# jrobine/actor-critic

Hardware: AMD Instinct MI355X
Metric: env-steps/sec (whole node) + ACKTR update ms, Breakout 84x84x4 (higher is better)
Workload: dtype fp32

## Files before the change

actor-critic_amd/actorcritic/_lib.py:

```python

import ctypes
import os

import torch

_HERE = os.path.dirname(os.path.abspath(__file__))
LIB_PATH = os.path.join(os.path.dirname(_HERE), 'libacmi.so')
if os.environ.get('ACMI_LIB'):
    LIB_PATH = os.environ['ACMI_LIB']

c_int = ctypes.c_int
c_i64 = ctypes.c_int64
c_u32 = ctypes.c_uint32
c_float = ctypes.c_float
c_vp = ctypes.c_void_p


class AcmiError(RuntimeError):
    """A libacmi entry point returned a non-zero status."""


class Net(ctypes.Structure):
    _fields_ = [('num_actions', c_int), ('conv3_filters', c_int), ('params', c_vp), ('conv_prep', c_vp),
                ('gemm_mode', c_int), ('forward_mode', c_int), ('conv_stats_mode', c_int)]
# ... 102 lines not shown
    'acmi_diag_segments': (c_int, [c_vp, c_vp, c_vp, c_int, c_vp, c_vp, c_vp]),
    'acmi_a2c_loss_ws_floats': (c_i64, [c_int]),
    'acmi_a2c_loss': (c_int, [c_vp, c_int, c_vp, c_vp, c_vp, c_vp, c_int, c_int, c_float, c_float, c_float,
                              c_vp, c_int, c_vp, c_vp, c_vp]),
    'acmi_ppo_loss_ws_floats': (c_i64, [c_int]),
    'acmi_ppo_loss': (c_int, [c_vp, c_int, c_vp, c_vp, c_vp, c_vp, c_vp, c_vp, c_int, c_int, c_float, c_float,
                              c_float, c_float, c_float, c_vp, c_int, c_vp, c_vp, c_vp, c_vp]),
    'acmi_gather_rows': (c_int, [c_vp, c_i64, c_i64, c_vp, c_i64, c_vp, c_i64, c_int, ctypes.POINTER(c_vp),
                                 ctypes.POINTER(c_vp), c_vp, c_vp]),
    'acmi_backward_ws_floats': (c_i64, [c_int, c_int, c_int]),
    'acmi_backward': (c_int, [ctypes.POINTER(Net), c_vp, c_i64, c_int, ctypes.POINTER(Acts),
                              ctypes.POINTER(Bwd), c_vp, c_vp, c_vp, c_i64, c_vp]),
    'acmi_kfac_output_stats': (c_int, [ctypes.POINTER(Net), c_int, ctypes.POINTER(Acts), ctypes.POINTER(Bwd),
                                       c_u32, c_u32, c_u32, c_vp, c_vp, c_i64, c_vp]),
    'acmi_backward_stacked': (c_int, [ctypes.POINTER(Net), c_vp, c_i64, c_int, ctypes.POINTER(Acts),
                                      ctypes.POINTER(Bwd), c_vp, c_vp, c_vp, c_i64, ctypes.POINTER(Bwd), c_u32, c_u32,
                                      c_u32, c_vp, c_i64, c_vp]),
    'acmi_kfac_output_stats_finish': (c_int, [ctypes.POINTER(Net), c_int, ctypes.POINTER(Acts), ctypes.POINTER(Bwd),
                                              c_vp, c_vp, c_i64, c_vp]),
    'acmi_debug_ws_flushes': (c_int, []),
    'acmi_debug_convt2': (c_int, [ctypes.POINTER(Net), c_int, c_vp, c_vp, c_vp, c_vp, c_int, c_vp, c_vp, c_vp, c_vp,
                                  c_vp]),
    'acmi_debug_convt2_form': (c_int, [c_int]),
    'acmi_kfac_ema': (c_int, [c_vp, c_vp, c_vp, c_i64, c_float, c_float, c_float, c_vp]),
    'acmi_kfac_inverse_layout': (c_int, [c_int, c_int, ctypes.POINTER(c_i64), ctypes.POINTER(c_i64)]),
    'acmi_kfac_inverse_floats': (c_i64, [c_int, c_int]),
    'acmi_kfac_inverse_ws_doubles': (c_i64, [c_int, c_int]),
    'acmi_kfac_inverse': (c_int, [c_int, c_int, c_vp, c_float, c_int, c_vp, c_vp, c_vp]),
    'acmi_kfac_eig_ws_doubles': (c_i64, [c_int, c_int]),
    'acmi_kfac_eigvals': (c_int, [c_int, c_int, c_vp, c_vp, c_vp, c_vp]),
    'acmi_kfac_step_ws_floats': (c_i64, [c_int, c_int]),
    'acmi_kfac_step': (c_int, [c_int, c_int, c_vp, c_vp, c_vp, c_vp, c_float, c_float, c_float, c_vp, c_vp,
                               c_vp, c_vp]),
    'acmi_opt_ws_floats': (c_i64, [c_i64]),
    'acmi_momentum_apply': (c_int, [c_vp, c_vp, c_vp, c_i64, c_float, c_float, c_float, c_vp, c_vp, c_vp]),
    'acmi_rmsprop_apply': (c_int, [c_vp, c_vp, c_vp, c_vp, c_i64, c_float, c_float, c_float, c_float, c_float,
                                   c_vp, c_vp, c_vp]),
    'acmi_adam_apply': (c_int, [c_vp, c_vp, c_vp, c_vp, c_i64, c_float, c_float, c_float, c_float, c_float,
                                c_vp, c_vp, c_vp]),
    'acmi_env_reset': (c_int, [ctypes.POINTER(EnvState), c_int, c_int, c_u32, c_vp, c_i64, c_vp]),
    'acmi_env_step': (c_int, [ctypes.POINTER(EnvState), c_int, c_int, c_u32, c_vp, c_vp, c_i64, c_vp, c_i64,
                              c_vp, c_vp, c_vp, c_i64, c_vp]),
    'acmi_game_state_ints': (c_int, []),
    'acmi_game_state_bytes': (c_i64, []),
    'acmi_game_reset': (c_int, [ctypes.POINTER(GameState), c_int, c_int, c_u32, c_vp, c_i64, c_vp]),
    'acmi_game_step': (c_int, [ctypes.POINTER(GameState), c_int, c_int, c_u32, c_vp, c_vp, c_i64, c_vp, c_i64,
# ... 99 lines not shown
```

actor-critic_amd/csrc/gemm.hpp:

```cpp
#pragma once

#include <algorithm>
#include <type_traits>

#include "gemm_ops.hpp"


namespace acmi {

typedef float f32x16 __attribute__((ext_vector_type(16)));

template <int BM, int BN, int BK, int WTM, int WTN>
struct Tile {
  static constexpr int WAVES_M = BM / (32 * WTM);
  static constexpr int WAVES_N = BN / (32 * WTN);
  static_assert(WAVES_M * WAVES_N == 4, "4 waves per block");
  static_assert(BK % 2 == 0 && BK % 4 == 0, "");
  static_assert((BM * BK / 4) % 256 == 0 && (BN * BK / 4) % 256 == 0,
                "staging must split evenly over 256 threads");
};

template <class T, class = void>
struct has_vec4 : std::false_type {};
template <class T>
// ... 424 lines not shown
    if (relu) v = fmaxf(v, 0.f);
    out[(long long)i * ld + j] = v;
  }
};

template <bool MASK = false>
struct EpiReluGrad {
  float* out;
  const float* act;
  long long ld;
  unsigned* amax = nullptr;
  __device__ __forceinline__ float aux(int i, int j) const {
    const long long e = (long long)i * ld + j;
    if constexpr (MASK) return (float)((reinterpret_cast<const uint32_t*>(act)[e >> 5] >> (e & 31)) & 1u);
    else return act[e];
  }
  __device__ __forceinline__ float store(int i, int j, float v, float x) const {
    const float o = x > 0.f ? v : 0.f;
    out[(long long)i * ld + j] = o;
    return o;
  }
};

template <int IH, int IW, int S, int CIN, bool MASK = false>
struct EpiConvT {
  static constexpr bool VEC4 = true;
  static constexpr bool LDS_T = true;
  static_assert(CIN % 4 == 0, "channel runs of 4");
  float* out;
  const float* act;
  unsigned* amax = nullptr;
  __device__ __forceinline__ long long offset(int i, int j) const {
    constexpr int PH = IH / S, PW = IW / S, L = PH * PW;
    const uint32_t img = (uint32_t)j / L;
    const uint32_t p = (uint32_t)j - img * L;
    const uint32_t ihp = p / PW;
    const uint32_t iwp = p - ihp * PW;
    const int ph = i / (S * CIN);
    const int rem = i - ph * (S * CIN);
    const int pw = rem / CIN;
    const int ci = rem - pw * CIN;
    return (((long long)img * IH + (S * ihp + ph)) * IW + (S * iwp + pw)) * CIN + ci;
  }
  __device__ __forceinline__ float4 aux4(int i0, int j) const {
    const long long e = offset(i0, j);
    if constexpr (MASK) {
// ... 114 lines not shown
```

actor-critic_amd/csrc/gemm3.hpp:

```cpp
#pragma once

#include "f16x2.hpp"
#include "gemm.hpp"
#include "symred3.hpp"

namespace acmi {

template <int RB>
__device__ __forceinline__ int sw_rows(int slot, int k) {
  const int q = k & 3;
  if constexpr (RB >= 256) return slot ^ (8 * q);
  else if constexpr (RB == 128) return slot ^ (8 * ((q >> 1) & 1));
  else return slot;
}

template <int BK>
__device__ __forceinline__ int sw_kc(int c, int i) {
  if constexpr (BK == 16) return c ^ ((i >> 3) & 1);
  else return c ^ ((i >> 2) & 3);
}

template <int BM, int BN, int BK, int NP = 3>
constexpr int gemm3_lds_bytes() {
  return 2 * NP * (BM + BN) * BK * 2;
// ... 26 lines not shown
    *reinterpret_cast<uint2*>(s + off) = h;
    *reinterpret_cast<uint2*>(s + PART + off) = m;
    if constexpr (NP == 3) *reinterpret_cast<uint2*>(s + 2 * PART + off) = l;
  }
  __device__ __forceinline__ static int frag_off(int lane, int ks, int x0) {
    if constexpr (KC) {
      const int x = x0 + (lane & 31);
      return x * RB + 16 * sw_kc<BK>(2 * ks + (lane >> 5), x);
    } else {
      const int q = (lane >> 2) & 3, p = lane & 3, g = (lane >> 4) & 1, kh = lane >> 5;
      const int k = 16 * ks + 8 * kh + q;
      return k * RB + 8 * sw_rows<RB>((x0 >> 2) + 4 * g + p, k);
    }
  }
  __device__ __forceinline__ static bf16x8 frag(const char* part, int off) {
    if constexpr (KC) {
      return __builtin_bit_cast(bf16x8, *reinterpret_cast<const uint4*>(part + off));
    } else {
      return cat8(ds_tr16(part + off), ds_tr16(part + off + 4 * RB));
    }
  }
};

template <int BM, int BN, int BK, int WTM, int WTN, bool SPLITK, bool COLSUM, class OpA, class OpB,
          class Epi, bool F16 = false>
__global__ __launch_bounds__(256)
__attribute__((amdgpu_waves_per_eu(gemm3_blocks_per_cu<BM, BN, BK, 3>())))
void gemm3_kernel(OpA opA, OpB opB, Epi epi, int I, int J, int K, int k_chunk, int sym_cols,
                  const unsigned* amax_a = nullptr, const unsigned* amax_b = nullptr) {
  using TL = Tile<BM, BN, BK, WTM, WTN>;
  static_assert(BK == 16 || BK == 32, "BK 16 or 32");
  static_assert(!COLSUM || !OpB::KCONTIG, "column sums need an i-contiguous B");
  constexpr int NP = F16 ? 2 : 3;
  using IA = X3Image<OpA::KCONTIG, BM, BK, NP>;
  using IB = X3Image<OpB::KCONTIG, BN, BK, NP>;
  float sa = 1.f, sb = 1.f;
  if constexpr (F16) {
    sa = f16x2_scale_of_bits(amax_a);
    sb = f16x2_scale_of_bits(amax_b);
  }
  int bx = blockIdx.x, by = blockIdx.y, bz = blockIdx.z;
  if constexpr (SPLITK) {
    const int tx = (I + BM - 1) / BM, ty = (J + BN - 1) / BN;
    const int ssym = sym_cols > 0 ? sym_cols / BN : 0;
    int live = 0;
    for (int x = 0; x < tx; ++x) live += ty - min(x * BM / BN, ssym);
    const int total = gridDim.x;
    const int b = blockIdx.x;
    const int xcd = b & 7, base = total >> 3, rem = total & 7;
    const int l = xcd * base + min(xcd, rem) + (b >> 3);
// ... 214 lines not shown
    __syncthreads();
    if (bx == 0 && wm == 0) {
#pragma unroll
      for (int tn = 0; tn < WTN; ++tn) {
        const int c = wn * WTN * 32 + tn * 32 + (lane & 31);
        float t = 0.f;
        for (int r = 0; r < KT; ++r) t += cs[r * BN + c];
        const int j = j0 + c;
        if (lane < 32 && j < J) epi.colsum(j, t);
      }
    }
    __syncthreads();
  }

  if constexpr (F16) {
    const float inv = 1.0f / (sa * sb);
#pragma unroll
    for (int a = 0; a < WTM; ++a)
#pragma unroll
      for (int b = 0; b < WTN; ++b)
#pragma unroll
        for (int r = 0; r < 16; ++r) acc[a][b][r] *= inv;
  }
  if constexpr (has_ldst<Epi>::value && 2 * (IA::BYTES + IB::BYTES) >= 4 * 32 * 36 * 4) {
    __syncthreads();
    store_tile_lds<WTM, WTN>(epi, acc, i0 + wm * WTM * 32, j0 + wn * WTN * 32, lane,
                             reinterpret_cast<float*>(lds) + wave * 32 * 36, I, J);
  } else {
    store_tile<WTM, WTN>(epi, acc, i0 + wm * WTM * 32, j0 + wn * WTN * 32, lane, I, J);
  }
}

template <int BM, int BN, int BK, int WTM, int WTN, bool SPLITK, bool COLSUM, class OpA, class OpB,
          class Epi>
inline void launch_gemm3(const OpA& a, const OpB& b, const Epi& e, int I, int J, int K, int zdim,
                         int k_chunk, hipStream_t s, int sym_cols = 0) {
  dim3 grid(cdiv(I, BM), cdiv(J, BN), zdim);
  if (SPLITK) grid = dim3(live_tiles<BM, BN>(I, J, sym_cols) * zdim);
  hipLaunchKernelGGL((gemm3_kernel<BM, BN, BK, WTM, WTN, SPLITK, COLSUM, OpA, OpB, Epi>), grid,
                     dim3(256), 0, s, a, b, e, I, J, K, k_chunk, sym_cols, nullptr, nullptr);
}

template <int BM, int BN, int BK, int WTM, int WTN, class OpA, class OpB, class Epi>
inline void launch_gemm3_f16(const OpA& a, const OpB& b, const Epi& e, int I, int J, int K,
                             const unsigned* amax_a, const unsigned* amax_b, hipStream_t s) {
  hipLaunchKernelGGL((gemm3_kernel<BM, BN, BK, WTM, WTN, false, false, OpA, OpB, Epi, true>),
                     dim3(cdiv(I, BM), cdiv(J, BN), 1), dim3(256), 0, s, a, b, e, I, J, K, 0, 0, amax_a,
// ... 24 lines not shown
```

actor-critic_amd/csrc/net.hip:

```cpp
#include <math.h>
#include <stdlib.h>
#include <stdarg.h>
#include <stdio.h>
#include <string.h>

#include <atomic>
#include <vector>

#include "gemm.hpp"
#include "gemm3.hpp"
#include "conv1u8.hpp"
#include "convt3.hpp"
#include "convfwd3.hpp"
#include "band.hpp"
#include "tower.hpp"
#include "fc4roll.hpp"
#include "convt2.hpp"
#include "stepper.hpp"
#include "towersplit.hpp"

namespace acmi {

static int s_gemm_mode = [] {
  const char* e = getenv("ACMI_GEMM");
// ... 150 lines not shown
  const float4 g4 = *reinterpret_cast<const float4*>(g);
  const float gv = g[4];
  const float4* w4 = reinterpret_cast<const float4*>(wpi + j0 * 4);
  const float4 x = *reinterpret_cast<const float4*>(a4 + q * 4);
  float o[4];
#pragma unroll
  for (int e = 0; e < 4; ++e) {
    const float4 w = w4[e];
    float acc = __builtin_fmaf(g4.x, w.x, 0.f);
    acc = __builtin_fmaf(g4.y, w.y, acc);
    acc = __builtin_fmaf(g4.z, w.z, acc);
    acc = __builtin_fmaf(g4.w, w.w, acc);
    o[e] = __builtin_fmaf(gv, wv[j0 + e], acc);
  }
  float4 r;
  r.x = o[0] * (float)(x.x > 0.f);
  r.y = o[1] * (float)(x.y > 0.f);
  r.z = o[2] * (float)(x.z > 0.f);
  r.w = o[3] * (float)(x.w > 0.f);
  if (ok) *reinterpret_cast<float4*>(d4 + q * 4) = r;
  if (amax) block_amax256(amax, ok ? absmax4f(r) : 0.f);
}

static bool masks_ok(const acmi_acts_t* a) { return (a->m1 && a->m2 && a->m3) || (!a->m1 && !a->m2 && !a->m3); }

inline int roundup4(int x) { return (x + 3) & ~3; }


}

#include "forward.hpp"
#include "splitk.hpp"

namespace acmi {

static hipEvent_t* dx_done_event() {
  static hipEvent_t ev[64] = {};
  int dev = 0;
  if (hipGetDevice(&dev) != hipSuccess || dev < 0 || dev >= 64) return nullptr;
  if (!ev[dev] && hipEventCreateWithFlags(&ev[dev], hipEventDisableTiming) != hipSuccess) {
    ev[dev] = nullptr;
    return nullptr;
  }
  return &ev[dev];
}
template <int C3>
static int dx_chain_pre(const Layout& L, const float* P, int B, const acmi_acts_t* a,
                        const acmi_bwd_t* bw, const float* dhead, int ldh,
                        hipStream_t s, const char* prep, unsigned* dxs) {
  ACMI_REQUIRE(dxs, ACMI_ERR_ARG, "dx_chain: no scratch");
  ACMI_REQUIRE(hipMemsetAsync(dxs, 0, kBandScratch * sizeof(unsigned), s) == hipSuccess, ACMI_ERR_HIP,
               "dx_chain: scratch reset failed");
  if (L.A == 4 && ldh % 4 == 0 && (uintptr_t)(P + L.off[8]) % 16 == 0 && (uintptr_t)dhead % 16 == 0)
    hipLaunchKernelGGL(heads_dx4_kernel, dim3(cdiv((long long)B * 128, 256)), dim3(256), 0, s, dhead,
                       ldh, B, P + L.off[8], P + L.off[10], a->a4, bw->d4, dxs + kBsMaxD4);
  else
    hipLaunchKernelGGL(heads_dx_kernel, dim3(cdiv((long long)B * 128, 256)), dim3(256), 0, s, dhead,
                       ldh, B, P + L.off[8], P + L.off[10], L.A, a->a4, bw->d4, dxs + kBsMaxD4);
  const unsigned* hdr = prep ? reinterpret_cast<const unsigned*>(prep + TowerPrep<C3>::HDR) : nullptr;
  const unsigned* w3max = hdr ? hdr + kTowMaxW3 : dxs + kBsMaxW3;
  const unsigned* w4max = hdr ? hdr + kTowMaxW4 : dxs + kBsMaxW4;
  if (!hdr && g_gemm_mode == ACMI_GEMM_X3) {
    hipLaunchKernelGGL(absmax_kernel, dim3(16), dim3(256), 0, s, P + L.off[4], (long long)576 * C3,
                       dxs + kBsMaxW3);
    hipLaunchKernelGGL(absmax_kernel, dim3(64), dim3(256), 0, s, P + L.off[6], (long long)49 * C3 * 512,
                       dxs + kBsMaxW4);
  }
  {
    const int K3 = 49 * C3;
    RowsAsK<DenseRows> opA{DenseRows{bw->d4, 512, B, 512}};
    MatTK<true> opB{P + L.off[6], 512, 512, K3};
    auto run = [&](auto epi) {
      if (g_gemm_mode == ACMI_GEMM_X3)
        launch_gemm3_f16<128, 64, 32, 2, 1>(opA, opB, epi, B, K3, 512, dxs + kBsMaxD4, w4max, s);
      else
        launch_mm<64, 128, 32, 1, 2, false, false, 16>(opA, opB, epi, B, K3, 512, 1, 0, s);
    };
    prof_begin(ACMI_PROF_FC4_DX, s);
    if (a->m3) run(EpiReluGrad<true>{bw->d3, reinterpret_cast<const float*>(a->m3), K3, dxs + kBsMaxD3});
    else run(EpiReluGrad<false>{bw->d3, a->a3, K3, dxs + kBsMaxD3});
    prof_end(ACMI_PROF_FC4_DX, s);
  }
  {
    const char* ct3p = prep ? prep + TowerPrep<C3>::BYTES + CT2::BYTES + fc4_prep_bytes(49 * C3) : nullptr;
    using Src = ConvTRows<9, 9, 3, 3, 1, C3>;
    using W = ConvTWeights<3, 3, 1, 64, C3>;
    W opA{P + L.off[4]};
    RowsAsK<Src> opB{Src{bw->d3, B * Src::L}};
    auto run = [&](auto epi) {
      if (g_gemm_mode == ACMI_GEMM_X3)
        launch_convt_x3<9, 9, 3, 3, 1, 64, C3, 256>(P + L.off[4], ct3p, bw->d3, B, epi, w3max, dxs + kBsMaxD3, s);
      else
        launch_mm<64, 128, 16, 1, 2, false, false, 16>(opA, opB, epi, W::N, B * Src::L, Src::COLS, 1, 0, s);
    };
    prof_begin(ACMI_PROF_CONV3_DX, s);
    if (a->m2) run(EpiConvT<9, 9, 1, 64, true>{bw->d2, reinterpret_cast<const float*>(a->m2), dxs + kBsMaxD2});
    else run(EpiConvT<9, 9, 1, 64>{bw->d2, a->a2, dxs + kBsMaxD2});
    prof_end(ACMI_PROF_CONV3_DX, s);
  }
  ACMI_LAUNCH_CHECK("dx_chain");
  return ACMI_OK;
}

static std::atomic<int> g_convt2_form{-1};
static bool convt2_use_resident(int B, bool gram) {
  const int f = g_convt2_form.load(std::memory_order_relaxed);
  return f < 0 ? convt2_resident_default(B, gram) : f != 0;
}

template <int C3>
static int dx_conv2(const Layout& L, const float* P, int B, const acmi_acts_t* a, const acmi_bwd_t* bw,
                    hipStream_t s, const char* prep, float* gram_part, bool* gram_done, unsigned* dxs) {
  if (gram_done) *gram_done = false;
  {
    using Src = ConvTRows<20, 20, 4, 4, 2, 64>;
    using W = ConvTWeights<4, 4, 2, 32, 64>;
    W opA{P + L.off[2]};
    RowsAsK<Src> opB{Src{bw->d2, B * Src::L}};
    const float* act1 = a->m1 ? reinterpret_cast<const float*>(a->m1) : a->a1;
    prof_begin(ACMI_PROF_CONV2_DX, s);
    const char* p2 = prep ? prep + TowerPrep<C3>::BYTES : nullptr;
    if (p2 && g_gemm_mode == ACMI_GEMM_X3) {
      auto go = [&](auto GRAMc, auto MASKc) {
        constexpr bool GR = decltype(GRAMc)::value, MK = decltype(MASKc)::value;
        if (convt2_use_resident(B, GR))
          hipLaunchKernelGGL((convt2_resident_kernel<GR, MK>), dim3(convt2_resident_blocks(B)), dim3(CT2R::THREADS),
                             0, s, p2, bw->d2, act1, GR ? nullptr : bw->d1, B, GR ? gram_part : nullptr,
                             dxs + kBsMaxD2, GR ? nullptr : dxs + kBsMaxD1, convt2_resident_teams(B));
        else if (GR)
          hipLaunchKernelGGL((convt2_kernel<GR, MK>), dim3(convt2_gram_blocks(B)), dim3(256), 0, s, p2, bw->d2,
                             act1, nullptr, B, gram_part, dxs + kBsMaxD2, nullptr);
// ... 8 lines not shown
        else go(T{}, F{});
        if (gram_done) *gram_done = true;
      } else {
        if (a->m1) go(F{}, T{});
        else go(F{}, F{});
      }
    } else if (a->m1) {
      launch_mm<128, 128, 16, 2, 2, false, false, 16>(
          opA, opB, EpiConvT<20, 20, 2, 32, true>{bw->d1, act1, dxs + kBsMaxD1}, W::N, B * Src::L, Src::COLS, 1, 0, s);
    } else {
      launch_mm<128, 128, 16, 2, 2, false, false, 16>(opA, opB, EpiConvT<20, 20, 2, 32>{bw->d1, act1, dxs + kBsMaxD1},
                                                      W::N, B * Src::L, Src::COLS, 1, 0, s);
    }
    prof_end(ACMI_PROF_CONV2_DX, s);
  }
  ACMI_LAUNCH_CHECK("dx_conv2");
  return ACMI_OK;
}

template <int C3>
static int dx_chain(const Layout& L, const float* P, int B, const acmi_acts_t* a,
                    const acmi_bwd_t* bw, const float* dhead, int ldh,
                    hipStream_t s, const char* prep = nullptr, float* gram_part = nullptr,
                    bool* gram_done = nullptr, unsigned* dxs = nullptr) {
  const int rc = dx_chain_pre<C3>(L, P, B, a, bw, dhead, ldh, s, prep, dxs);
  if (rc) return rc;
  return dx_conv2<C3>(L, P, B, a, bw, s, prep, gram_part, gram_done, dxs);
}

template <int C3>
static int backward_impl(const Layout& L, const float* P, const uint8_t* obs,
                         long long img_stride, int B, const acmi_acts_t* a,
                         const acmi_bwd_t* bw, float* grads, float* astat,
                         float* ws, long long ws_cap, hipStream_t s, const char* prep,
                         bool dx_done = false) {
  const bool st = astat != nullptr;
  const bool fuse_c1 = st && g_gemm_mode == ACMI_GEMM_X3;
  unsigned* bscr = reinterpret_cast<unsigned*>(ws);
  const long long prefix = bwd_prefix_floats(B);
  float* part = ws + prefix;
  const long long avail = ws_cap - prefix;
  const bool band = band_on(st);
  int rc = ACMI_OK;
  if (!dx_done) {
    rc = dx_chain<C3>(L, P, B, a, bw, bw->dhead, bw->ldh, s, prep, nullptr, nullptr, bscr);
    if (rc) return rc;
    hipEvent_t* ev = dx_done_event();
    ACMI_REQUIRE(ev && hipEventRecord(*ev, s) == hipSuccess, ACMI_ERR_HIP, "acmi_backward: dX event record failed");
// ... 37 lines not shown
                     ra, grads + L.off[4], C3, nullptr, st ? astat + L.stat_off[2] : nullptr);
  if (rc) return rc;
  ra.flush();
  if (band)
    rc = band_layer(a->a1, 20, 20, 32, 4, 4, 2, bw->d2, 64, B, part, avail, grads + L.off[2],
                    astat + L.stat_off[1], 1.f, a1b, bscr + kBsMaxD2, s, ACMI_PROF_CONV2_WGRAD);
  else
    rc = wgrad_layer(ConvRows<float, 20, 20, 32, 4, 4, 2>{a->a1, 400 * 32, B * 81}, 512, 81LL * B, bw->d2, 64, 64,
                     st, ra, grads + L.off[2], 64, nullptr, st ? astat + L.stat_off[1] : nullptr,
                     ACMI_PROF_CONV2_WGRAD);
  if (rc) return rc;
  ra.flush();
  if (!fuse_c1)
    rc = wgrad_layer(ConvRows<uint8_t, 84, 84, 4, 8, 8, 4>{obs, (uint32_t)img_stride, B * 400}, 256, 400LL * B,
                     bw->d1, 32, 32, false, ra, grads + L.off[0], 32, nullptr, nullptr, ACMI_PROF_CONV1_WGRAD,
                     1.0f / 255.0f);
  if (rc) return rc;
  ra.flush();
  ACMI_LAUNCH_CHECK("wgrad_layer");
  return ACMI_OK;
}

template <bool MASKED>
__global__ void sampled_head_grad_kernel(const float* logits, int ld, int B, int A, uint32_t seed, uint32_t row0,
                                         uint32_t ctr, float* g, int ldg, const uint32_t* legal) {
  const int m = blockIdx.x * blockDim.x + threadIdx.x;
  if (m >= B) return;
  const float* z = logits + (long long)m * ld;
  const uint32_t lg = MASKED ? legal_bits(legal[m], A) : 0xFFFFFFFFu;
  const RowMaxSum ms = row_max_sum<MASKED>(z, A, lg);
  const float mx = ms.mx, se = ms.se;
  const uint32_t h = key4(seed, 0u, ctr, row0 + (uint32_t)m);
  const float u = u01(h);
  const float target = u * se;
  float c = 0.f;
  int y = ms.last;
  for (int a = 0; a < A; ++a) {
    if (!legal_at<MASKED>(lg, a)) continue;
    c += expf(z[a] - mx);
    if (target < c) { y = a; break; }
  }
  float* gr = g + (long long)m * ldg;
  for (int a = 0; a < A; ++a)
    gr[a] = legal_at<MASKED>(lg, a) ? expf(z[a] - mx) / se - (a == y ? 1.f : 0.f) : 0.f;
  const float u1 = u01(mix32(h ^ 0x68e31da4U)) + (1.0f / 33554432.0f);
  const float u2 = u01(mix32(h ^ 0xb5297a4dU));
  const float eps = sqrtf(-2.f * logf(u1)) * cosf(6.2831853071795864f * u2);
  gr[A] = -eps;
  for (int a = A + 1; a < ldg; ++a) gr[a] = 0.f;
}
static void launch_sampled_head_grad(const float* logits, int ld, int B, int A, uint32_t seed, uint32_t row0,
                                     uint32_t ctr, float* g, int ldg, const uint32_t* legal, hipStream_t s) {
  const auto kern = legal ? sampled_head_grad_kernel<true> : sampled_head_grad_kernel<false>;
  hipLaunchKernelGGL(kern, dim3(cdiv(B, 128)), dim3(128), 0, s, logits, ld, B, A, seed, row0, ctr, g, ldg, legal);
}

template <int C3>
static int output_stats_impl(const Layout& L, const float* P, int B,
                             const acmi_acts_t* a, const acmi_bwd_t* bw,
                             uint32_t seed, uint32_t row0, uint32_t ctr,
                             float* gstat, float* ws, long long ws_cap,
                             hipStream_t s, const char* prep, int stage = 0,
                             const uint32_t* legal = nullptr) {
  const int ldg = (int)head_grad_ldg(L.A);
  unsigned* dxs = reinterpret_cast<unsigned*>(ws);
  float* ghead = ws + kBandScratch;
  const long long prefix = stats_prefix_floats(B, L.A);
  float* part = ws + prefix;
  const long long cap = ws_cap - prefix;
  bool g1_done = false;
  const bool g1_fits = (long long)convt2_gram_blocks(B) * 33 * 32 <= cap;
  int rc = ACMI_OK;
  if (stage == 0) {
    launch_sampled_head_grad(a->logits, a->ld_logits, B, L.A, seed, row0, ctr, ghead, ldg, legal, s);
    rc = dx_chain<C3>(L, P, B, a, bw, ghead, ldg, s, prep, g1_fits ? part : nullptr, &g1_done, dxs);
    if (rc) return rc;
  } else {
    g1_done = g1_fits && prep && g_gemm_mode == ACMI_GEMM_X3;
  }
  PartRanges<CovSet> ra{part, cap, s};
  if (g1_done) {
    const int nc = convt2_gram_blocks(B);
    const long long floats = (long long)nc * 33 * 32;
    const float* g1_part = ra.begin(floats);
    ra.add(g1_part, nc, 32, 32, gstat + L.stat_off[5 + 0], (int)(400LL * B), 1);
    rc = ra.end(floats);
    if (rc) return rc;
  }
  rc = gcov_layer(ghead, ldg, L.A + 1, B, L.A, ra, gstat + L.stat_off[5 + 4], gstat + L.stat_off[5 + 5], L.A);
  if (rc) return rc;
  rc = gcov_layer(bw->d4, 512, 512, B, 512, ra, gstat + L.stat_off[5 + 3], nullptr, -1, dxs + kBsMaxD4);
  if (rc) return rc;
  rc = gcov_layer(bw->d3, C3, C3, 49LL * B, C3, ra, gstat + L.stat_off[5 + 2]);
  if (rc) return rc;
  rc = gcov_layer(bw->d2, 64, 64, 81LL * B, 64, ra, gstat + L.stat_off[5 + 1], nullptr, -1, dxs + kBsMaxD2);
  if (rc) return rc;
  if (!g1_done) rc = gcov_layer(bw->d1, 32, 32, 400LL * B, 32, ra, gstat + L.stat_off[5 + 0]);
  if (rc) return rc;
  ra.flush();
  ACMI_LAUNCH_CHECK("G factor finalize");
  return ACMI_OK;
}

template <int C3>
static int backward_stacked_impl(const Layout& L, const float* P, const uint8_t* obs, long long img_stride, int B,
                                 const acmi_acts_t* a, const acmi_bwd_t* bw, float* grads, float* astat, float* ws,
                                 long long ws_cap, const acmi_bwd_t* bws, uint32_t seed, uint32_t row0, uint32_t ctr,
                                 float* wss, long long wss_cap, hipStream_t s, const char* prep) {
  unsigned* bscr = reinterpret_cast<unsigned*>(ws);
  int rc = dx_chain_pre<C3>(L, P, B, a, bw, bw->dhead, bw->ldh, s, prep, bscr);
  if (rc) return rc;
  const int ldg = (int)head_grad_ldg(L.A);
  unsigned* dxs = reinterpret_cast<unsigned*>(wss);
  float* ghead = wss + kBandScratch;
  float* part_s = wss + stats_prefix_floats(B, L.A);
  const long long cap_s = wss_cap - stats_prefix_floats(B, L.A);
  launch_sampled_head_grad(a->logits, a->ld_logits, B, L.A, seed, row0, ctr, ghead, ldg, nullptr, s);
  rc = dx_chain_pre<C3>(L, P, B, a, bws, ghead, ldg, s, prep, dxs);
  if (rc) return rc;
  const bool g1_fits = (long long)convt2_gram_blocks(B) * 33 * 32 <= cap_s;
  if (prep && g_gemm_mode == ACMI_GEMM_X3 && g1_fits) {
    const char* p2 = prep + TowerPrep<C3>::BYTES;
    const float* act1 = a->m1 ? reinterpret_cast<const float*>(a->m1) : a->a1;
    prof_begin(ACMI_PROF_CONV2_DX, s);
    if (a->m1)
      hipLaunchKernelGGL((convt2_kernel<true, true, true>), dim3(convt2_gram_blocks(B)), dim3(256), 0, s, p2, bw->d2,
                         act1, bw->d1, B, part_s, bscr + kBsMaxD2, bscr + kBsMaxD1, bws->d2, dxs + kBsMaxD2);
    else
      hipLaunchKernelGGL((convt2_kernel<true, false, true>), dim3(convt2_gram_blocks(B)), dim3(256), 0, s, p2, bw->d2,
                         act1, bw->d1, B, part_s, bscr + kBsMaxD2, bscr + kBsMaxD1, bws->d2, dxs + kBsMaxD2);
    prof_end(ACMI_PROF_CONV2_DX, s);
    ACMI_LAUNCH_CHECK("stacked conv2 dX");
  } else {
    rc = dx_conv2<C3>(L, P, B, a, bw, s, prep, nullptr, nullptr, bscr);
    if (rc) return rc;
    bool g1_done = false;
    rc = dx_conv2<C3>(L, P, B, a, bws, s, prep, g1_fits ? part_s : nullptr, &g1_done, dxs);
    if (rc) return rc;
  }
  {
    hipEvent_t* ev = dx_done_event();
    ACMI_REQUIRE(ev && hipEventRecord(*ev, s) == hipSuccess, ACMI_ERR_HIP, "acmi_backward: dX event record failed");
  }
// ... 452 lines not shown
  hipStream_t s = (hipStream_t)stream;
  const float* act1 = reinterpret_cast<const float*>(m1);
  if (mode == 0) {
    hipLaunchKernelGGL((convt2_kernel<false, true>), dim3(convt2_store_blocks(B)), dim3(256), 0, s, p2, d2a, act1, d1,
                       B, nullptr, d2max_a, d1max, nullptr, nullptr);
    hipLaunchKernelGGL((convt2_kernel<true, true>), dim3(convt2_gram_blocks(B)), dim3(256), 0, s, p2, d2b, act1,
                       nullptr, B, gram_part, d2max_b, nullptr, nullptr, nullptr);
  } else if (mode == 1) {
    hipLaunchKernelGGL((convt2_kernel<true, true, true>), dim3(convt2_gram_blocks(B)), dim3(256), 0, s, p2, d2a,
                       act1, d1, B, gram_part, d2max_a, d1max, d2b, d2max_b);
  } else {
    const dim3 grid(convt2_resident_blocks(B)), block(CT2R::THREADS);
    hipLaunchKernelGGL((convt2_resident_kernel<false, true>), grid, block, 0, s, p2, d2a, act1, d1, B, nullptr,
                       d2max_a, d1max, convt2_resident_teams(B));
    hipLaunchKernelGGL((convt2_resident_kernel<true, true>), grid, block, 0, s, p2, d2b, act1, nullptr, B, gram_part,
                       d2max_b, nullptr, convt2_resident_teams(B));
  }
  ACMI_LAUNCH_CHECK("acmi_debug_convt2");
  return ACMI_OK;
}

int acmi_debug_convt2_form(int form) {
  return g_convt2_form.exchange(form < 0 ? -1 : form != 0, std::memory_order_relaxed);
}

int acmi_debug_ws_flushes(void) {
  return g_ws_flushes.exchange(0);
}

int acmi_selftest_plans(int max_k) {
  for (int K = 64; K <= max_k; K += 32) {
    SymPlan p;
    if (!sym_plan(K, 64, &p)) continue;
    const int J = K + 64;
    std::vector<unsigned char> cov((size_t)K * J, 0);
    std::vector<int> cs(J, 0);
    for (int g = 0; g < p.ngroups; ++g)
      for (int w = 0; w < 4; ++w) {
        if (p.g[g].wa[w] < 0) continue;
        const int a = p.g[g].base[p.g[g].wa[w]], b = p.g[g].base[p.g[g].wb[w]];
        if (a < 0 || b < 0 || a >= K) return K;
        for (int i = a; i < a + 64 && i < K; ++i)
          for (int j = b; j < b + 64 && j < J; ++j) cov[(size_t)i * J + j] = 1;
        if (a == 0)
          for (int j = b; j < b + 64 && j < J; ++j) cs[j]++;
      }
// ... 107 lines not shown
```

actor-critic_amd/csrc/splitk.hpp:

```cpp
#pragma once

#include <algorithm>
#include <atomic>
#include <type_traits>

#include "band.hpp"
#include "conv1u8.hpp"
#include "gemm.hpp"
#include "gemm3.hpp"

namespace acmi {

struct WgradDesc {
  const float* part;
  int nchunk;
  int I;
  int J;
  int kp;
  int cout;
  float* gradA;
  int nsplit;
  float* gradB;
  float* astat;
  int rows;
// ... 463 lines not shown
      launch_symred<16>(opB, epi, pl.sp, I, J, (int)rows, nc, ch, s);
    else if (with_stats)
      launch_mm<128, 128, 16, 2, 2, true, true, 16>(opA, opB, epi, I, J, (int)rows, nc, ch, s, K);
    else
      launch_mm<128, 32, 32, 1, 1, true, true, 32>(opA, opB, epi, I, J, (int)rows, nc, ch, s);
  } else {
    ACMI_REQUIRE(K == 256 && cout == 32 && ldy == 32, ACMI_ERR_ARG, "conv1 weight gradient shape");
    launch_conv1_wgrad_u8(src, dy, (int)rows, nc, ch, epi, s);
  }
  prof_end(site, s);
  const bool tiles = astat && nc <= kFinGroups;
  WgradDesc d{part, nc, I, J, kp, cout, gradA, nsplit, gradB, tiles ? nullptr : astat, (int)rows, wscale};
  ra.add(d, 0);
  if (tiles) {
    d.astat = astat;
    ra.add(d, 1);
  }
  ACMI_LAUNCH_CHECK("wgrad_layer");
  return ra.end(pl.floats);
}

static int gcov_layer(const float* g, int ld, int n, long long rows, int sub,
                      PartRanges<CovSet>& ra, float* out, float* out_v = nullptr, int v_index = -1,
                      const unsigned* gmax = nullptr) {
  hipStream_t s = ra.s;
  float* part = ra.begin(gcov_need(n, rows));
  int np, nc;
  if (n <= 32) {
    np = 32;
    long long ch;
    gram_plan(rows, &nc, &ch);
    ACMI_REQUIRE((long long)nc * (np + 1) * np <= ra.room(), ACMI_ERR_WS, "gcov workspace too small");
    hipLaunchKernelGGL(gram_small_kernel<32>, dim3(nc), dim3(256), 0, s, g, ld, n, rows, ch, part);
  } else {
    const GcovPlan pl = gcov_plan(n, rows);
    np = pl.np;
    nc = pl.nc;
    DenseRows src{g, ld, (int)rows, np};
    RowsAsI<DenseRows> op{src};
    ACMI_REQUIRE(pl.floats <= ra.room(), ACMI_ERR_WS, "gcov workspace too small");
    EpiPartial epi{part, np, np};
    if (gmax && g_gemm_mode == ACMI_GEMM_X3)
      launch_gemm3_f16_splitk<64, 64, 16, 1, 1>(op, op, epi, np, np, (int)rows, nc, (int)pl.ch, gmax, gmax, s, np);
    else
      launch_mm<64, 64, 32, 1, 1, true, false, 16>(op, op, epi, np, np, (int)rows, nc, pl.ch, s, np);
  }
  ra.add(part, nc, np, sub, out, (int)rows, nc <= 64 ? (sub >= 64 ? 3 : 0) : 1);
  if (out_v) ra.add(part, nc, np, 1, out_v, (int)rows, 2, v_index);
  ACMI_LAUNCH_CHECK("gcov_layer");
  return ra.end((long long)nc * (np + 1) * np);
}

static long long bwd_partial_floats(int B, int A, int C3) {
  long long m = 0;
  const long long rowsL[5] = {400LL * B, 81LL * B, 49LL * B, B, B};
  const int Ks[5] = {256, 512, 576, 49 * C3, 512};
  const int co[5] = {32, 64, C3, 512, A + 1};
  for (int l = 0; l < 5; ++l) {
    for (int mode : {ACMI_GEMM_F32, ACMI_GEMM_X3})
      m = std::max(m, wgrad_plan(Ks[l], co[l], true, rowsL[l], false, mode).floats);
    for (int mode : {ACMI_GEMM_F32, ACMI_GEMM_X3})
      m = std::max(m, wgrad_plan(Ks[l], co[l], false, rowsL[l], l == 0, mode).floats);
    if (co[l] <= 64) {
      int nc;
      long long ch;
      gram_plan(rowsL[l], &nc, &ch);
      const long long np = co[l] <= 32 ? 32 : 64;
      m = std::max(m, nc * (np + 1) * np);
    }
// ... 15 lines not shown
```

include/acmi.h:

```cpp
#ifndef ACMI_H_
#define ACMI_H_

#include <stdint.h>

#ifdef __cplusplus
extern "C" {
#endif

#define ACMI_ABI_VERSION 4

enum {
  ACMI_OK = 0,
  ACMI_ERR_ARG = -1,
  ACMI_ERR_HIP = -2,
  ACMI_ERR_WS = -3,
};

typedef void* acmi_stream_t;

const char* acmi_last_error(void);
int acmi_abi_version(void);
int acmi_abi_struct_sizes(int64_t* sizes, int n);

#define ACMI_GEMM_F32 0
// ... 378 lines not shown
typedef struct acmi_rollout_game_io {
  acmi_rollout_io_t io;
  acmi_game_state_t state;
  const uint8_t* games;
  acmi_game_rules_t rules;
  uint8_t* truncated;
  int32_t* bad_envs;
  int32_t* pend;
} acmi_rollout_game_io_t;
int acmi_game_pend_ints(void);
int64_t acmi_rollout_game_io_bytes(void);
int acmi_rollout_step_games(const acmi_net_t* net, const uint8_t* obs,
                            int64_t img_stride, int B, const acmi_acts_t* acts,
                            int64_t act_img_stride, const acmi_rollout_game_io_t* io,
                            const uint32_t* legal, acmi_stream_t stream);

int acmi_selftest_plans(int max_k);
int acmi_debug_ws_flushes(void);
int acmi_debug_convt2(const acmi_net_t* net, int mode, const float* d2a, const float* d2b,
                      const uint32_t* m1, float* d1, int B, float* gram_part,
                      const uint32_t* d2max_a, const uint32_t* d2max_b, uint32_t* d1max,
                      acmi_stream_t stream);
int acmi_debug_convt2_form(int form);

int acmi_gemm_f32(const float* A, const float* B, float* C, int M, int N,
                  int K, acmi_stream_t stream);

#define ACMI_PROF_CONV1_WGRAD 1
#define ACMI_PROF_CONV2_WGRAD 2
#define ACMI_PROF_CONV1_FWD 3
#define ACMI_PROF_CONV1_AFACTOR 4
#define ACMI_PROF_CONV2_DX 5
#define ACMI_PROF_FC4_DX 6
#define ACMI_PROF_CONV3_DX 7
int acmi_prof_enable(int site, int capacity);
int acmi_prof_collect(double* total_ms, int* count);

#ifdef __cplusplus
}
#endif
#endif
```

Baseline: 3.023 million.

## Fuse K-FAC gradient Gram statistics into head-grad and fc4 dx epilogues

Computes the head-gradient Gram matrix inside the sampled head-gradient kernel, and the d3 (conv3 output gradient) Gram inside the fc4 input-gradient GEMM epilogue using split-bf16 MFMAs on the freshly produced tile. This avoids two separate gcov passes that re-read d3 and the head gradients from memory, along with their launches. In exchange the fused fc4 kernel is forced to a 128x64 tile at lower occupancy (waves_per_eu 2) and needs extra LDS and workspace ranges. The fusion is controlled by a debug toggle that defaults to on. Profiling sites are also added.

```diff
diff --git a/actor-critic_amd/actorcritic/_lib.py b/actor-critic_amd/actorcritic/_lib.py
--- a/actor-critic_amd/actorcritic/_lib.py
+++ b/actor-critic_amd/actorcritic/_lib.py
@@ -148,6 +148,7 @@
     'acmi_debug_convt2': (c_int, [ctypes.POINTER(Net), c_int, c_vp, c_vp, c_vp, c_vp, c_int, c_vp, c_vp, c_vp, c_vp,
                                   c_vp]),
     'acmi_debug_convt2_form': (c_int, [c_int]),
+    'acmi_debug_gstats_fused': (c_int, [c_int]),
     'acmi_kfac_ema': (c_int, [c_vp, c_vp, c_vp, c_i64, c_float, c_float, c_float, c_vp]),
     'acmi_kfac_inverse_layout': (c_int, [c_int, c_int, ctypes.POINTER(c_i64), ctypes.POINTER(c_i64)]),
     'acmi_kfac_inverse_floats': (c_i64, [c_int, c_int]),
diff --git a/actor-critic_amd/csrc/gemm.hpp b/actor-critic_amd/csrc/gemm.hpp
--- a/actor-critic_amd/csrc/gemm.hpp
+++ b/actor-critic_amd/csrc/gemm.hpp
@@ -470,6 +470,16 @@
   }
 };
 
+template <bool MASK, int C>
+struct EpiReluGradGram : EpiReluGrad<MASK> {
+  static constexpr int GRAM_C = C;
+  float* gpart;
+};
+template <class T, class = void>
+struct has_gram : std::false_type {};
+template <class T>
+struct has_gram<T, std::void_t<decltype(T::GRAM_C)>> : std::true_type {};
+
 template <int IH, int IW, int S, int CIN, bool MASK = false>
 struct EpiConvT {
   static constexpr bool VEC4 = true;
diff --git a/actor-critic_amd/csrc/gemm3.hpp b/actor-critic_amd/csrc/gemm3.hpp
--- a/actor-critic_amd/csrc/gemm3.hpp
+++ b/actor-critic_amd/csrc/gemm3.hpp
@@ -72,10 +72,123 @@
   }
 };
 
+template <int C>
+constexpr int gram_tile_lds_bytes() {
+  return (C == 64 ? 2 * 2 * 2 * 3 * 64 * 16 : 0) + C * C * 4;
+}
+template <int WTM, class Epi, class Acc>
+__device__ __forceinline__ void store_tile_gram(const Epi& epi, const Acc& acc, int ib, int jb, int lane, int wm,
+                                                int wn, char* lds, int I, int J, long long block) {
+  constexpr int C = Epi::GRAM_C;
+  static_assert(WTM == 2 && (C == 32 || C == 64), "128 x 64 tiles, 32 or 64 channels");
+  const int khalf = lane >> 5, c = lane & 31, tid = threadIdx.x;
+  const int j = jb + c;
+  float x[WTM][16], o[WTM][16];
+#pragma unroll
+  for (int tm = 0; tm < WTM; ++tm)
+#pragma unroll
+    for (int r = 0; r < 16; ++r)
+      x[tm][r] = epi.aux(min(ib + tm * 32 + (r & 3) + 8 * (r >> 2) + 4 * khalf, I - 1), min(j, J - 1));
+  float am = 0.f;
+#pragma unroll
+  for (int tm = 0; tm < WTM; ++tm)
+#pragma unroll
+    for (int r = 0; r < 16; ++r) {
+      const int i = ib + tm * 32 + (r & 3) + 8 * (r >> 2) + 4 * khalf;
+      o[tm][r] = 0.f;
+      if (i < I && j < J) {
+        o[tm][r] = epi.store(i, j, acc[tm][0][r], x[tm][r]);
+        am = fmaxf(am, fabsf(o[tm][r]));
+      }
+    }
+  amax_publish(epi.amax, am, lane);
+
+  bf16x8 f[WTM][2][3];
+#pragma unroll
+  for (int tm = 0; tm < WTM; ++tm)
+#pragma unroll
+    for (int s = 0; s < 2; ++s) {
+      const float* v = &o[tm][8 * s];
+      uint4 hh, mm, ll;
+      split3(v[0], v[1], hh.x, mm.x, ll.x);
+      split3(v[2], v[3], hh.y, mm.y, ll.y);
+      split3(v[4], v[5], hh.z, mm.z, ll.z);
+      split3(v[6], v[7], hh.w, mm.w, ll.w);
+      f[tm][s][0] = __builtin_bit_cast(bf16x8, hh);
+      f[tm][s][1] = __builtin_bit_cast(bf16x8, mm);
+      f[tm][s][2] = __builtin_bit_cast(bf16x8, ll);
+    }
+  f32x16 g0, g1;
+#pragma unroll
+  for (int r = 0; r < 16; ++r) g0[r] = 0.f, g1[r] = 0.f;
+#pragma unroll
+  for (int tm = 0; tm < WTM; ++tm)
+#pragma unroll
+    for (int s = 0; s < 2; ++s) g0 = mfma_x3(f[tm][s], f[tm][s], g0);
+
+  constexpr int EXB = gram_tile_lds_bytes<C>() - C * C * 4;
+  float* red = reinterpret_cast<float*>(lds + EXB);
+  if constexpr (C == 64) {
+    uint4* ex = reinterpret_cast<uint4*>(lds) + (long long)wm * (WTM * 2 * 3 * 64) + lane;
+    if (wn == 1) {
+#pragma unroll
+      for (int tm = 0; tm < WTM; ++tm)
+#pragma unroll
+        for (int s = 0; s < 2; ++s)
+#pragma unroll
+          for (int p = 0; p < 3; ++p) ex[((tm * 2 + s) * 3 + p) * 64] = __builtin_bit_cast(uint4, f[tm][s][p]);
+    }
+    __syncthreads();
+    if (wn == 0) {
+#pragma unroll
+      for (int tm = 0; tm < WTM; ++tm)
+#pragma unroll
+        for (int s = 0; s < 2; ++s) {
+          bf16x8 b[3];
+#pragma unroll
+          for (int p = 0; p < 3; ++p) b[p] = __builtin_bit_cast(bf16x8, ex[((tm * 2 + s) * 3 + p) * 64]);
+          g1 = mfma_x3(f[tm][s], b, g1);
+        }
+    }
+#pragma unroll
+    for (int w = 0; w < 2; ++w) {
+      if (wm == w) {
+#pragma unroll
+        for (int r = 0; r < 16; ++r) {
+          const int e = (32 * wn + (r & 3) + 8 * (r >> 2) + 4 * khalf) * 64 + 32 * wn + c;
+          red[e] = (w ? red[e] : 0.f) + g0[r];
+          if (wn == 0) red[e + 32] = (w ? red[e + 32] : 0.f) + g1[r];
+        }
+      }
+      __syncthreads();
+    }
+    float* out = epi.gpart + block * (65 * 64);
+    for (int e = tid; e < 64 * 64; e += 256) {
+      const int i = e >> 6, jj = e & 63;
+      out[e] = (i >= 32 && jj < 32) ? red[jj * 64 + i] : red[e];
+    }
+  } else {
+    const int wave = 2 * wm + wn;
+#pragma unroll
+    for (int w = 0; w < 4; ++w) {
+      if (wave == w) {
+#pragma unroll
+        for (int r = 0; r < 16; ++r) {
+          const int e = ((r & 3) + 8 * (r >> 2) + 4 * khalf) * 32 + c;
+          red[e] = (w ? red[e] : 0.f) + g0[r];
+        }
+      }
+      __syncthreads();
+    }
+    float* out = epi.gpart + block * (33 * 32);
+    for (int e = tid; e < 32 * 32; e += 256) out[e] = red[e];
+  }
+}
+
 template <int BM, int BN, int BK, int WTM, int WTN, bool SPLITK, bool COLSUM, class OpA, class OpB,
           class Epi, bool F16 = false>
 __global__ __launch_bounds__(256)
-__attribute__((amdgpu_waves_per_eu(gemm3_blocks_per_cu<BM, BN, BK, 3>())))
+__attribute__((amdgpu_waves_per_eu(gemm3_blocks_per_cu<BM, BN, BK, has_gram<Epi>::value ? 2 : 3>())))
 void gemm3_kernel(OpA opA, OpB opB, Epi epi, int I, int J, int K, int k_chunk, int sym_cols,
                   const unsigned* amax_a = nullptr, const unsigned* amax_b = nullptr) {
   using TL = Tile<BM, BN, BK, WTM, WTN>;
@@ -336,7 +449,12 @@
 #pragma unroll
         for (int r = 0; r < 16; ++r) acc[a][b][r] *= inv;
   }
-  if constexpr (has_ldst<Epi>::value && 2 * (IA::BYTES + IB::BYTES) >= 4 * 32 * 36 * 4) {
+  if constexpr (has_gram<Epi>::value) {
+    static_assert(BM == 128 && BN == 64 && WTN == 1 && !SPLITK && !COLSUM, "the Gram epilogue's tile");
+    static_assert(gram_tile_lds_bytes<Epi::GRAM_C>() <= 2 * (IA::BYTES + IB::BYTES), "Gram epilogue LDS");
+    store_tile_gram<WTM>(epi, acc, i0 + wm * WTM * 32, j0 + wn * 32, lane, wm, wn, lds, I, J,
+                         (long long)by * gridDim.x + bx);
+  } else if constexpr (has_ldst<Epi>::value && 2 * (IA::BYTES + IB::BYTES) >= 4 * 32 * 36 * 4) {
     __syncthreads();
     store_tile_lds<WTM, WTN>(epi, acc, i0 + wm * WTM * 32, j0 + wn * WTN * 32, lane,
                              reinterpret_cast<float*>(lds) + wave * 32 * 36, I, J);
diff --git a/actor-critic_amd/csrc/net.hip b/actor-critic_amd/csrc/net.hip
--- a/actor-critic_amd/csrc/net.hip
+++ b/actor-critic_amd/csrc/net.hip
@@ -196,6 +196,8 @@
   if (amax) block_amax256(amax, ok ? absmax4f(r) : 0.f);
 }
 
+inline int fc4_gram_blocks(int B, int C3) { return cdiv(B, 128) * cdiv(49 * C3, 64); }
+
 static bool masks_ok(const acmi_acts_t* a) { return (a->m1 && a->m2 && a->m3) || (!a->m1 && !a->m2 && !a->m3); }
 
 inline int roundup4(int x) { return (x + 3) & ~3; }
@@ -221,7 +223,7 @@
 template <int C3>
 static int dx_chain_pre(const Layout& L, const float* P, int B, const acmi_acts_t* a,
                         const acmi_bwd_t* bw, const float* dhead, int ldh,
-                        hipStream_t s, const char* prep, unsigned* dxs) {
+                        hipStream_t s, const char* prep, unsigned* dxs, float* g3_part = nullptr) {
   ACMI_REQUIRE(dxs, ACMI_ERR_ARG, "dx_chain: no scratch");
   ACMI_REQUIRE(hipMemsetAsync(dxs, 0, kBandScratch * sizeof(unsigned), s) == hipSuccess, ACMI_ERR_HIP,
                "dx_chain: scratch reset failed");
@@ -251,8 +253,22 @@
         launch_mm<64, 128, 32, 1, 2, false, false, 16>(opA, opB, epi, B, K3, 512, 1, 0, s);
     };
     prof_begin(ACMI_PROF_FC4_DX, s);
-    if (a->m3) run(EpiReluGrad<true>{bw->d3, reinterpret_cast<const float*>(a->m3), K3, dxs + kBsMaxD3});
-    else run(EpiReluGrad<false>{bw->d3, a->a3, K3, dxs + kBsMaxD3});
+    if (g3_part) {
+      ACMI_REQUIRE(g_gemm_mode == ACMI_GEMM_X3, ACMI_ERR_ARG, "dx_chain: the fused d3 Gram needs x3 mode");
+      if (a->m3)
+        launch_gemm3_f16<128, 64, 32, 2, 1>(
+            opA, opB,
+            EpiReluGradGram<true, C3>{{bw->d3, reinterpret_cast<const float*>(a->m3), K3, dxs + kBsMaxD3}, g3_part}, B,
+            K3, 512, dxs + kBsMaxD4, w4max, s);
+      else
+        launch_gemm3_f16<128, 64, 32, 2, 1>(opA, opB,
+                                            EpiReluGradGram<false, C3>{{bw->d3, a->a3, K3, dxs + kBsMaxD3}, g3_part},
+                                            B, K3, 512, dxs + kBsMaxD4, w4max, s);
+    } else if (a->m3) {
+      run(EpiReluGrad<true>{bw->d3, reinterpret_cast<const float*>(a->m3), K3, dxs + kBsMaxD3});
+    } else {
+      run(EpiReluGrad<false>{bw->d3, a->a3, K3, dxs + kBsMaxD3});
+    }
     prof_end(ACMI_PROF_FC4_DX, s);
   }
   {
@@ -281,6 +297,8 @@
   const int f = g_convt2_form.load(std::memory_order_relaxed);
   return f < 0 ? convt2_resident_default(B, gram) : f != 0;
 }
+
+static std::atomic<int> g_gstats_fused{1};
 
 template <int C3>
 static int dx_conv2(const Layout& L, const float* P, int B, const acmi_acts_t* a, const acmi_bwd_t* bw,
@@ -335,8 +353,8 @@
 static int dx_chain(const Layout& L, const float* P, int B, const acmi_acts_t* a,
                     const acmi_bwd_t* bw, const float* dhead, int ldh,
                     hipStream_t s, const char* prep = nullptr, float* gram_part = nullptr,
-                    bool* gram_done = nullptr, unsigned* dxs = nullptr) {
-  const int rc = dx_chain_pre<C3>(L, P, B, a, bw, dhead, ldh, s, prep, dxs);
+                    bool* gram_done = nullptr, unsigned* dxs = nullptr, float* g3_part = nullptr) {
+  const int rc = dx_chain_pre<C3>(L, P, B, a, bw, dhead, ldh, s, prep, dxs, g3_part);
   if (rc) return rc;
   return dx_conv2<C3>(L, P, B, a, bw, s, prep, gram_part, gram_done, dxs);
 }
@@ -420,10 +438,9 @@
 }
 
 template <bool MASKED>
-__global__ void sampled_head_grad_kernel(const float* logits, int ld, int B, int A, uint32_t seed, uint32_t row0,
-                                         uint32_t ctr, float* g, int ldg, const uint32_t* legal) {
-  const int m = blockIdx.x * blockDim.x + threadIdx.x;
-  if (m >= B) return;
+__device__ __forceinline__ void sampled_head_grad_row(const float* logits, int ld, int m, int A, uint32_t seed,
+                                                      uint32_t row0, uint32_t ctr, float* g, int ldg,
+                                                      const uint32_t* legal) {
   const float* z = logits + (long long)m * ld;
   const uint32_t lg = MASKED ? legal_bits(legal[m], A) : 0xFFFFFFFFu;
   const RowMaxSum ms = row_max_sum<MASKED>(z, A, lg);
@@ -447,10 +464,60 @@
   gr[A] = -eps;
   for (int a = A + 1; a < ldg; ++a) gr[a] = 0.f;
 }
+template <bool MASKED, bool GRAM>
+__global__ void sampled_head_grad_kernel(const float* logits, int ld, int B, int A, uint32_t seed, uint32_t row0,
+                                         uint32_t ctr, float* g, int ldg, const uint32_t* legal, float* gpart) {
+  const int m = blockIdx.x * blockDim.x + threadIdx.x;
+  if constexpr (!GRAM) {
+    if (m >= B) return;
+    sampled_head_grad_row<MASKED>(logits, ld, m, A, seed, row0, ctr, g, ldg, legal);
+  } else {
+    __shared__ float rows[128][33];
+    const int n = A + 1;
+    if (m < B) sampled_head_grad_row<MASKED>(logits, ld, m, A, seed, row0, ctr, g, ldg, legal);
+    for (int a = 0; a < n; ++a) rows[threadIdx.x][a] = m < B ? g[(long long)m * ldg + a] : 0.f;
+    __syncthreads();
+    float* out = gpart + (long long)blockIdx.x * (33 * 32);
+    for (int e = threadIdx.x; e < n * n; e += 128) {
+      const int i = e / n, j = e - i * n;
+      if (i > j) continue;
+      float sum = 0.f;
+      for (int r = 0; r < 128; ++r) sum = __builtin_fmaf(rows[r][i], rows[r][j], sum);
+      out[i * 32 + j] = sum;
+      out[j * 32 + i] = sum;
+    }
+  }
+}
+inline int head_gram_blocks(int B) { return cdiv(B, 128); }
 static void launch_sampled_head_grad(const float* logits, int ld, int B, int A, uint32_t seed, uint32_t row0,
-                                     uint32_t ctr, float* g, int ldg, const uint32_t* legal, hipStream_t s) {
-  const auto kern = legal ? sampled_head_grad_kernel<true> : sampled_head_grad_kernel<false>;
-  hipLaunchKernelGGL(kern, dim3(cdiv(B, 128)), dim3(128), 0, s, logits, ld, B, A, seed, row0, ctr, g, ldg, legal);
+                                     uint32_t ctr, float* g, int ldg, const uint32_t* legal, hipStream_t s,
+                                     float* gpart = nullptr) {
+  const auto kern = gpart ? (legal ? sampled_head_grad_kernel<true, true> : sampled_head_grad_kernel<false, true>)
+                          : (legal ? sampled_head_grad_kernel<true, false> : sampled_head_grad_kernel<false, false>);
+  prof_begin(ACMI_PROF_HEAD_GRAD, s);
+  hipLaunchKernelGGL(kern, dim3(cdiv(B, 128)), dim3(128), 0, s, logits, ld, B, A, seed, row0, ctr, g, ldg, legal, gpart);
+  prof_end(ACMI_PROF_HEAD_GRAD, s);
+}
+
+struct GstatRanges {
+  bool g1_fits, gh_fused, g3_fused;
+  int gh_nc, g3_nc;
+  long long gh_off, gh_floats, g3_off, g3_floats;
+};
+static GstatRanges gstat_ranges(int B, int A, int C3, long long cap, const char* prep) {
+  GstatRanges r;
+  const long long g1 = (long long)convt2_gram_blocks(B) * 33 * 32;
+  r.g1_fits = g1 <= cap;
+  const bool fuse = prep && g_gemm_mode == ACMI_GEMM_X3 && g_gstats_fused.load(std::memory_order_relaxed);
+  r.gh_nc = head_gram_blocks(B);
+  r.g3_nc = fc4_gram_blocks(B, C3);
+  r.gh_floats = (long long)r.gh_nc * 33 * 32;
+  r.g3_floats = (long long)r.g3_nc * (C3 + 1) * C3;
+  r.gh_off = r.g1_fits ? g1 : 0;
+  r.gh_fused = fuse && A + 1 <= 32 && r.gh_off + r.gh_floats <= cap;
+  r.g3_off = r.gh_off + (r.gh_fused ? r.gh_floats : 0);
+  r.g3_fused = fuse && r.g3_off + r.g3_floats <= cap;
+  return r;
 }
 
 template <int C3>
@@ -467,15 +534,22 @@
   float* part = ws + prefix;
   const long long cap = ws_cap - prefix;
   bool g1_done = false;
-  const bool g1_fits = (long long)convt2_gram_blocks(B) * 33 * 32 <= cap;
+  const GstatRanges gr = gstat_ranges(B, L.A, C3, cap, prep);
+  const bool g1_fits = gr.g1_fits, gh_fused = gr.gh_fused, g3_fused = gr.g3_fused;
+  const int gh_nc = gr.gh_nc, g3_nc = gr.g3_nc;
+  const long long gh_floats = gr.gh_floats, gh_off = gr.gh_off, g3_floats = gr.g3_floats, g3_off = gr.g3_off;
   int rc = ACMI_OK;
   if (stage == 0) {
-    launch_sampled_head_grad(a->logits, a->ld_logits, B, L.A, seed, row0, ctr, ghead, ldg, legal, s);
-    rc = dx_chain<C3>(L, P, B, a, bw, ghead, ldg, s, prep, g1_fits ? part : nullptr, &g1_done, dxs);
+    launch_sampled_head_grad(a->logits, a->ld_logits, B, L.A, seed, row0, ctr, ghead, ldg, legal, s,
+                             gh_fused ? part + gh_off : nullptr);
+    rc = dx_chain<C3>(L, P, B, a, bw, ghead, ldg, s, prep, g1_fits ? part : nullptr, &g1_done, dxs,
+                      g3_fused ? part + g3_off : nullptr);
     if (rc) return rc;
   } else {
     g1_done = g1_fits && prep && g_gemm_mode == ACMI_GEMM_X3;
   }
+  ACMI_REQUIRE(!(gh_fused || g3_fused) || g1_done == g1_fits, ACMI_ERR_ARG,
+               "internal: conv2's input gradient declined the Gram the ranges were planned with");
   PartRanges<CovSet> ra{part, cap, s};
   if (g1_done) {
     const int nc = convt2_gram_blocks(B);
@@ -485,13 +559,33 @@
     rc = ra.end(floats);
     if (rc) return rc;
   }
-  rc = gcov_layer(ghead, ldg, L.A + 1, B, L.A, ra, gstat + L.stat_off[5 + 4], gstat + L.stat_off[5 + 5], L.A);
-  if (rc) return rc;
+  if (gh_fused) {
+    const float* p = ra.begin(gh_floats);
+    ACMI_REQUIRE(p == part + gh_off, ACMI_ERR_ARG, "internal: the head Gram's range moved");
+    ra.add(p, gh_nc, 32, L.A, gstat + L.stat_off[5 + 4], B, gh_nc <= 64 ? 0 : 1);
+    ra.add(p, gh_nc, 32, 1, gstat + L.stat_off[5 + 5], B, 2, L.A);
+    rc = ra.end(gh_floats);
+    if (rc) return rc;
+  }
+  if (g3_fused) {
+    const float* p = ra.begin(g3_floats);
+    ACMI_REQUIRE(p == part + g3_off, ACMI_ERR_ARG, "internal: the d3 Gram's range moved");
+    ra.add(p, g3_nc, C3, C3, gstat + L.stat_off[5 + 2], (int)(49LL * B), g3_nc <= 64 ? (C3 >= 64 ? 3 : 0) : 1);
+    rc = ra.end(g3_floats);
+    if (rc) return rc;
+  }
+  if (!gh_fused) {
+    rc = gcov_layer(ghead, ldg, L.A + 1, B, L.A, ra, gstat + L.stat_off[5 + 4], gstat + L.stat_off[5 + 5], L.A, nullptr,
+                    ACMI_PROF_GCOV_HEADS);
+    if (rc) return rc;
+  }
   rc = gcov_layer(bw->d4, 512, 512, B, 512, ra, gstat + L.stat_off[5 + 3], nullptr, -1, dxs + kBsMaxD4);
   if (rc) return rc;
-  rc = gcov_layer(bw->d3, C3, C3, 49LL * B, C3, ra, gstat + L.stat_off[5 + 2]);
+  if (!g3_fused) rc = gcov_layer(bw->d3, C3, C3, 49LL * B, C3, ra, gstat + L.stat_off[5 + 2], nullptr, -1, nullptr,
+                                 ACMI_PROF_GCOV_D3);
   if (rc) return rc;
-  rc = gcov_layer(bw->d2, 64, 64, 81LL * B, 64, ra, gstat + L.stat_off[5 + 1], nullptr, -1, dxs + kBsMaxD2);
+  rc = gcov_layer(bw->d2, 64, 64, 81LL * B, 64, ra, gstat + L.stat_off[5 + 1], nullptr, -1, dxs + kBsMaxD2,
+                  ACMI_PROF_GCOV_D2);
   if (rc) return rc;
   if (!g1_done) rc = gcov_layer(bw->d1, 32, 32, 400LL * B, 32, ra, gstat + L.stat_off[5 + 0]);
   if (rc) return rc;
@@ -513,10 +607,12 @@
   float* ghead = wss + kBandScratch;
   float* part_s = wss + stats_prefix_floats(B, L.A);
   const long long cap_s = wss_cap - stats_prefix_floats(B, L.A);
-  launch_sampled_head_grad(a->logits, a->ld_logits, B, L.A, seed, row0, ctr, ghead, ldg, nullptr, s);
-  rc = dx_chain_pre<C3>(L, P, B, a, bws, ghead, ldg, s, prep, dxs);
+  const GstatRanges gr = gstat_ranges(B, L.A, C3, cap_s, prep);
+  launch_sampled_head_grad(a->logits, a->ld_logits, B, L.A, seed, row0, ctr, ghead, ldg, nullptr, s,
+                           gr.gh_fused ? part_s + gr.gh_off : nullptr);
+  rc = dx_chain_pre<C3>(L, P, B, a, bws, ghead, ldg, s, prep, dxs, gr.g3_fused ? part_s + gr.g3_off : nullptr);
   if (rc) return rc;
-  const bool g1_fits = (long long)convt2_gram_blocks(B) * 33 * 32 <= cap_s;
+  const bool g1_fits = gr.g1_fits;
   if (prep && g_gemm_mode == ACMI_GEMM_X3 && g1_fits) {
     const char* p2 = prep + TowerPrep<C3>::BYTES;
     const float* act1 = a->m1 ? reinterpret_cast<const float*>(a->m1) : a->a1;
@@ -1015,6 +1111,10 @@
 
 int acmi_debug_convt2_form(int form) {
   return g_convt2_form.exchange(form < 0 ? -1 : form != 0, std::memory_order_relaxed);
+}
+
+int acmi_debug_gstats_fused(int on) {
+  return g_gstats_fused.exchange(on != 0, std::memory_order_relaxed);
 }
 
 int acmi_debug_ws_flushes(void) {
diff --git a/actor-critic_amd/csrc/splitk.hpp b/actor-critic_amd/csrc/splitk.hpp
--- a/actor-critic_amd/csrc/splitk.hpp
+++ b/actor-critic_amd/csrc/splitk.hpp
@@ -509,10 +509,11 @@
 
 static int gcov_layer(const float* g, int ld, int n, long long rows, int sub,
                       PartRanges<CovSet>& ra, float* out, float* out_v = nullptr, int v_index = -1,
-                      const unsigned* gmax = nullptr) {
+                      const unsigned* gmax = nullptr, int site = 0) {
   hipStream_t s = ra.s;
   float* part = ra.begin(gcov_need(n, rows));
   int np, nc;
+  prof_begin(site, s);
   if (n <= 32) {
     np = 32;
     long long ch;
@@ -532,6 +533,7 @@
     else
       launch_mm<64, 64, 32, 1, 1, true, false, 16>(op, op, epi, np, np, (int)rows, nc, pl.ch, s, np);
   }
+  prof_end(site, s);
   ra.add(part, nc, np, sub, out, (int)rows, nc <= 64 ? (sub >= 64 ? 3 : 0) : 1);
   if (out_v) ra.add(part, nc, np, 1, out_v, (int)rows, 2, v_index);
   ACMI_LAUNCH_CHECK("gcov_layer");
diff --git a/include/acmi.h b/include/acmi.h
--- a/include/acmi.h
+++ b/include/acmi.h
@@ -424,6 +424,7 @@
                       const uint32_t* d2max_a, const uint32_t* d2max_b, uint32_t* d1max,
                       acmi_stream_t stream);
 int acmi_debug_convt2_form(int form);
+int acmi_debug_gstats_fused(int on);
 
 int acmi_gemm_f32(const float* A, const float* B, float* C, int M, int N,
                   int K, acmi_stream_t stream);
@@ -435,6 +436,10 @@
 #define ACMI_PROF_CONV2_DX 5
 #define ACMI_PROF_FC4_DX 6
 #define ACMI_PROF_CONV3_DX 7
+#define ACMI_PROF_HEAD_GRAD 8
+#define ACMI_PROF_GCOV_HEADS 9
+#define ACMI_PROF_GCOV_D3 10
+#define ACMI_PROF_GCOV_D2 11
 int acmi_prof_enable(int site, int capacity);
 int acmi_prof_collect(double* total_ms, int* count);
 
```

New measurement: 3.043 million (median of 6 runs). No clear change (+0.7%).
